# ActiveVisionLab/NeFeS

Measured on AMD Instinct MI355X. Metric: rays/s (fwd+bwd) at 640x480x(64+128) samples, 8x256 MLP, higher is better.
Workload: dtype f32; 1 GPU; BASELINE configs[1]: 7-Scenes-stairs geometry, 64+128 samples, 8x256 MLP + 16-ch feature head; 640x480, random seed-0 weights, fwd + bwd to the 3x4 pose; parallelism=rows/1

## Files before the change

include/nefes_hip.h:

```cpp
#ifndef NEFES_HIP_H
#define NEFES_HIP_H
#include <stddef.h>
#include <stdint.h>

#ifdef __cplusplus
extern "C" {
#endif

#define NEFES_ABI_VERSION 20
#define NEFES_BLOB_FORMAT 17

#define NEFES_E_BADARG (-1)
#define NEFES_E_UNSUPPORTED (-2)
#define NEFES_E_BADBLOB (-3)

typedef struct NefesNetDesc {
    int32_t width;
    int32_t feat_dim;
    int32_t has_transient;
    int32_t xyz_encoding;
    int32_t fold_final;
} NefesNetDesc;
#define NEFES_XYZ_FREQ10 0
#define NEFES_XYZ_EXTERNAL32 1
// ... 13 lines not shown
} NefesBlobInfo;

#define NEFES_COMP_TRANSIENT 1u
#define NEFES_COMP_STATIC_ONLY 2u
#define NEFES_COMP_SIGMA_ONLY 4u
#define NEFES_COMP_WHITE_BKGD 8u
#define NEFES_COMP_FEAT_WEIGHTS_ONLY 16u

#define NEFES_FIELD_SIGMA 0
#define NEFES_FIELD_STATIC 1
#define NEFES_FIELD_FULL 2

int nefes_version(void);

int nefes_blob_info(const NefesNetDesc* desc, NefesBlobInfo* info);
size_t nefes_stream_slab_bytes(const NefesNetDesc* desc, int stream);
int nefes_pack_weights(const NefesNetDesc* desc, const float* const* tensors, int n_tensors, void* blob,
                       size_t blob_bytes);
int nefes_pack_map(const NefesNetDesc* desc, uint32_t* map, size_t n_entries, int64_t* tensor_elems_out);
int nefes_pack_h3_plan(const NefesNetDesc* desc, int32_t* plan, size_t n_ints, size_t* needed);
int nefes_pack_device(const float* flat, int64_t n_params, const uint32_t* map, int64_t n_entries, const int32_t* plan,
                      int n_jobs, int32_t* scratch, void* blob, void* stream);

int nefes_raygen_fwd(int H, int W, float focal, const float* c2w, int row0, int nrows, float* rays_o, float* rays_d,
                     float* viewdirs, void* stream);
size_t nefes_raygen_bwd_workspace(int n_rays);
int nefes_raygen_bwd(int H, int W, float focal, const float* c2w, int row0, int nrows, const float* g_rays_o,
                     const float* g_rays_d, const float* g_viewdirs, void* workspace, float* g_c2w, void* stream);
int nefes_raygen_k_fwd(int H, int W, const float* intr, const float* c2w, int row0, int nrows, float* rays_o, float* rays_d,
                       float* viewdirs, void* stream);
// ... 280 lines not shown
```

nefes_amd/csrc/field_fwd_h3.hip:

```cpp
#include "field_h3_instances.h"
#ifdef NEFES_TU_W128
#define NEFES_SLAB_KIB 16
#else
#define NEFES_SLAB_KIB 32
#endif
#include <stdio.h>
#include <stdlib.h>
#if defined(NEFES_TU_W128) || !defined(H3_NO_ACC_READ_ASM)
#define NEFES_ASM_READS_ACC
#define NEFES_FENCE_TILES
#endif
#if defined(NEFES_TU_W128)
#define NEFES_ACC_VGPR_FORM
#endif

#ifndef NEFES_FWD_CONSUMER_BIAS
#define NEFES_FWD_CONSUMER_BIAS 1
#endif
#include "field_common.h"
#include "../../include/nefes_hip.h"

#include "field_x6.h"
#include "hashgrid.h"
#if !defined(NEFES_TU_W128) && !defined(H3_NO_ACC_READ_ASM)
#define H3_ACC_READ_ASM
#endif
#include "field_h3.h"
#define NEFES_H3_SLOTS 2

struct FieldFwdH3Args {
    const char* stream;
    const float* bias;
// ... 4 lines not shown
    const float* pts;
    const float* xyz_enc;
    const float* viewdirs;
    float* raw_t;
    uint32_t* masks;
    int N, S, R, C;
    long long M;
    int n_tiles;
    uint32_t s_magic, s_shift;
    float* acts;
    int rows;
    int z_row;
    const float2* hg_table;
    HgGeom hg;
    int gout;
};

template <int NT, int T0, int NX>
__device__ __forceinline__ void train_save_h3(float* tile_base, uint32_t voff, int row0, const f32x16 (&X)[NX], float inv) {
    float* p = tile_base + (size_t)(row0 >> 5) * 4096 + voff;
#pragma unroll
    for (int t = 0; t < NT; ++t)
#pragma unroll
        for (int r = 0; r < 16; ++r) {
#ifndef NEFES_TRAIN_NO_STORES
            __builtin_nontemporal_store(X[T0 + t][r] * inv, &p[t * 4096 + nefes_rho(0, r) * 16]);
#endif
        }
}

template <int MODEF, int ENC, int W = 256, int NTR = 1, bool TRAIN = false, bool FH = false>
__global__ __launch_bounds__(256, W == 128 ? 2 : 1) void field_fwd_h3_kernel(FieldFwdH3Args a) {
    constexpr bool FOLD = MODEF == NEFES_FIELD_FULL_FOLD;
    constexpr int MODE = FOLD ? NEFES_FIELD_FULL : MODEF;
    static_assert(NEFES_SLAB_KIB == (W == 128 ? NEFES_H3_FWD_SLAB_KIB_128 : NEFES_H3_FWD_SLAB_KIB), "ring slab size != the packer's for this width");
    static_assert(!FOLD || (MODE != NEFES_FIELD_SIGMA && !TRAIN), "the fold serves the head products of frozen networks");
    constexpr int NTW = W / 32, NTH = W / 64;
    constexpr int ES = ENC != NEFES_XYZ_FREQ10 ? NEFES_X_STEPS : NEFES_E_STEPS;
    constexpr int MW = 8 * (W / 64) + 4 * (W / 128), WT = (NTW + 1) / 2, WH = (NTH + 1) / 2;
    constexpr int NSEG = MODE == NEFES_FIELD_SIGMA ? NEFES_H3F_SIG + 1
                         : (MODE == NEFES_FIELD_STATIC ? NEFES_H3F_N_STATIC : (FOLD ? NEFES_H3FF_N : NEFES_H3F_N));
    extern __shared__ __attribute__((aligned(16))) char smem[];
    char* ring_base = smem;
    float* bias_lds = (float*)(smem + NEFES_H3_SLOTS * NEFES_SLAB_BYTES);
    float* e_lds = bias_lds + ((a.bias_floats + 63) / 64) * 64 + (threadIdx.x >> 6) * (ES * 64) + (threadIdx.x & 63);
    const int lane = threadIdx.x & 63;
    const int wave = __builtin_amdgcn_readfirstlane(threadIdx.x >> 6);
    const int j = lane & 31, h = lane >> 5;
    for (uint32_t i = threadIdx.x; i < a.bias_floats; i += 256) bias_lds[i] = a.bias[i];
    HgGeom* hg_lds = (HgGeom*)(bias_lds + ((a.bias_floats + 63) / 64) * 64 + 4 * ES * 64);
    if constexpr (ENC == NEFES_XYZ_HASHGRID_FUSED) {
        if (threadIdx.x == 0) *hg_lds = a.hg;
    }
    StagedRing ring;
    ring.init(a.stream, a.n_slabs, ring_base, wave, lane);
    const char* ring_lane = ring_base + lane * 16;
    const char* bias_half = (const char*)bias_lds + 16 * h;
    const int* tab_i = (const int*)(bias_lds + a.scale_off);
    const float* tab_f = bias_lds + a.scale_off;
    auto wexp = [&](int seg) { return tab_i[nefes_h3_tab_exp(nefes_h3f_seg(FOLD, seg))]; };
    auto rowb = [&](int seg) { return tab_f[nefes_h3_tab_bound(nefes_h3f_seg(FOLD, seg))]; };
    auto bmax = [&](int blk) { return tab_f[nefes_h3_tab_bias(NSEG, nefes_h3f_bias(FOLD, blk))]; };
    ring.prime(ring_lane);
    constexpr int B_SIG = 8 * W, B_FINAL = B_SIG + 32, B_DIR = B_FINAL + (FOLD ? 0 : W), B_RGB = B_DIR + W / 2,
                  B_T0 = B_RGB + 32 * NTR, B_T1 = B_T0 + W / 2, B_T2 = B_T1 + W / 2, B_TH = B_T2 + W / 2;
#pragma unroll 1
    for (int tile = blockIdx.x; tile < a.n_tiles; tile += gridDim.x) {
        auto locate = [&](uint32_t& m, uint32_t& ray, uint32_t& smp) {
            const uint32_t m_raw = (uint32_t)tile * 128u + (uint32_t)(wave * 32 + j);
            const bool ok = m_raw < (uint32_t)a.M;
            m = ok ? m_raw : (uint32_t)a.M - 1u;
            ray = a.s_magic ? __umulhi(m, a.s_magic) >> a.s_shift : m;
// ... 59 lines not shown
        };
        auto bias_at = [&](int off_floats, int es) { return BiasInitScaled{bias_half + off_floats * 4, pow2i(es)}; };
        constexpr bool CB = !TRAIN && W == 256 && NEFES_FWD_CONSUMER_BIAS;
        float2 nbias;
        f32x16 A[NTW], B[NTW];
        uint32_t bits[WT];
        auto clear_bits = [&]() {
#pragma unroll
            for (int w = 0; w < WT; ++w) bits[w] = 0u;
        };
        constexpr bool CAP = MODE != NEFES_FIELD_SIGMA;
        auto tau_of = [&](float M, int ew) {
            const int t = pick_exp(M);
            return t < 100 - ew ? t : 100 - ew;
        };
        auto sigma_head = [&](const f32x16 (&X)[NTW], int es_x, int tau_x) {
            f32x16 sg[1];
            float mdummy = 0.f;
            const int es = tau_x + wexp(NEFES_H3F_SIG);
            if constexpr (CB) {
                const char* bp8 = bias_half + 7 * W * 4;
                nbias = ReluBiasSplitH<false, NTW, WT>::prime(bp8);
                mma_run_h3<1, W / 16, 0, true>(ring, ring_lane, ReluBiasSplitH<false, NTW, WT>{X, bits, pow2i(tau_x - es_x), mdummy, bp8, pow2i(es_x), nbias},
                                               bias_at(B_SIG, es), sg);
            } else
            mma_run_h3<1, W / 16, 0, true>(ring, ring_lane, ReluSplitH<false, NTW, WT>{X, bits, pow2i(tau_x - es_x), mdummy},
                                           bias_at(B_SIG, es), sg);
            float* col = raw_col();
            if (col && h == 0) {
                const int ch = (MODE == NEFES_FIELD_SIGMA) ? 0 : 3 + a.C;
                __builtin_nontemporal_store(softplus_ref(sg[0][0] * pow2i(-es)), &col[(size_t)ch * a.S]);
            }
        };
        int es_a, es_b = 0;
        float M;
        {
            const int tau = tau_of(mE, wexp(NEFES_H3F_L1));
            es_a = tau + wexp(NEFES_H3F_L1);
            if constexpr (CB) mma_run_h3<NTW, ES / 8, 0, true>(ring, ring_lane, LdsSplitH{e_lds, pow2i(tau)}, ZeroInit{}, A);
            else mma_run_h3<NTW, ES / 8, 0, true>(ring, ring_lane, LdsSplitH{e_lds, pow2i(tau)}, bias_at(0, es_a), A);
            M = rowb(NEFES_H3F_L1) * mE + bmax(NEFES_H3BB_L1);
            save_trunk(1, A, es_a);
        }
#define NEFES_FWD_EVEN_LAYER(L1_, SEG1_)                                                                                       \
        clear_bits();                                                                                                          \
        {                                                                                                                      \
            const int ew = wexp(SEG1_), tau = tau_of(M, ew);                                                                   \
// ... 68 lines not shown
#pragma unroll
                for (int s = 0; s < NEFES_D_STEPS; ++s) __builtin_nontemporal_store(Dv[s], &pd[2 * s * 16]);
            }
            f32x16 dt[NDT];
            uint32_t bits2[WH];
            auto clear2 = [&]() {
#pragma unroll
                for (int w = 0; w < WH; ++w) bits2[w] = 0u;
            };
            struct Bias2 {
                BiasInitScaled a, b;
                __device__ __forceinline__ f32x16 operator()(int t) const { return t < NTH ? a(t) : b(t - NTH); }
            };
            int es_dt;
            if constexpr (FOLD) {
                sigma_head(B, es_b, tau_of(M, wexp(NEFES_H3F_SIG)));
                const int ew = wexp(NEFES_H3F_DT_H);
                const float mD = pair_max(array_max(Dv));
                const int tau = tau_of(fmaxf(M, mD), ew);
                const float rbh_ = rowb(NEFES_H3F_DT_H), rbd_ = rowb(NEFES_H3F_DT_D);
                const float bm_ = fmaxf(bmax(NEFES_H3BB_DIR), bmax(NEFES_H3BB_T0));
                float mx = 0.f;
                es_dt = tau + ew;
                clear_bits();
                if constexpr (CB) {
                    const char* bp8 = bias_half + 7 * W * 4;
                    nbias = ReluBiasSplitH<CAP, NTW, WT>::prime(bp8);
                    const ReluBiasSplitH<CAP, NTW, WT> src8{B, bits, pow2i(tau - es_b), mx, bp8, pow2i(es_b), nbias};
                    mma_run_h3<NDT, W / 16, 0, true>(ring, ring_lane, src8, Bias2{bias_at(B_DIR, es_dt), bias_at(B_T0, es_dt)}, dt);
                } else {
                    const ReluSplitH<CAP, NTW, WT> src8{B, bits, pow2i(tau - es_b), mx};
                    mma_run_h3<NDT, W / 16, 0, true>(ring, ring_lane, src8, Bias2{bias_at(B_DIR, es_dt), bias_at(B_T0, es_dt)}, dt);
                }
                mma_run_h3<NDT, 2, 0, false>(ring, ring_lane, ArraySplitH<16>{Dv, pow2i(tau)}, ZeroInit{}, dt);
                M = rbh_ * (pair_max(mx) * pow2i(-es_b)) + rbd_ * mD + bm_;
                put_masks(bits, WT);
            } else {
                const int ew = wexp(NEFES_H3F_DT_H);
                const float mD = pair_max(array_max(Dv));
                const int tau = tau_of(fmaxf(M, mD), ew);
                float mx = 0.f;
                es_dt = tau + ew;
                if constexpr (CB) {
                    const char* bpf = bias_half + B_FINAL * 4;
                    nbias = ReluBiasSplitH<false, 1, 1>::prime(bpf);
                    const IdentBiasSplitH<NTW> srcf{A, pow2i(tau - es_a), mx, bpf, pow2i(es_a), nbias};
                    if constexpr (FULL) mma_run_h3<NDT, W / 16, 0, true>(ring, ring_lane, srcf, Bias2{bias_at(B_DIR, es_dt), bias_at(B_T0, es_dt)}, dt);
                    else mma_run_h3<NDT, W / 16, 0, true>(ring, ring_lane, srcf, bias_at(B_DIR, es_dt), dt);
// ... 110 lines not shown
}

static void magic_div(uint32_t d, uint32_t& magic, uint32_t& shift) {
    if (d == 1) { magic = 0; shift = 0; return; }
    uint32_t l = 0;
    while ((1ull << l) < d) ++l;
    const uint64_t p = 31 + l;
    magic = (uint32_t)(((1ull << p) + d - 1) / d);
    shift = (uint32_t)(p - 32);
}

template <int MODE, int ENC, int W = 256, int NTR = 1, bool TRAIN = false, bool FH = false>
static int launch_h3(const FieldFwdH3Args& a, hipStream_t st) {
    constexpr int ES_ = ENC != NEFES_XYZ_FREQ10 ? NEFES_X_STEPS : NEFES_E_STEPS;
    const size_t lds = (size_t)NEFES_H3_SLOTS * NEFES_SLAB_BYTES + ((a.bias_floats + 63) / 64) * 256 + (size_t)4 * ES_ * 64 * 4
                       + (ENC == NEFES_XYZ_HASHGRID_FUSED ? 512 : 0);
    static_assert(sizeof(HgGeom) <= 512, "the level geometry's LDS slot");
    auto k = field_fwd_h3_kernel<MODE, ENC, W, NTR, TRAIN, FH>;
    hipError_t e = hipFuncSetAttribute((const void*)k, hipFuncAttributeMaxDynamicSharedMemorySize, (int)lds);
    if (e != hipSuccess) return (int)e;
    int dev = 0, cus = 256;
    (void)hipGetDevice(&dev);
    (void)hipDeviceGetAttribute(&cus, hipDeviceAttributeMultiprocessorCount, dev);
    const int per_cu = W == 128 ? 2 : 1;
    int grid = a.n_tiles < cus * per_cu ? a.n_tiles : cus * per_cu;
    if (const char* cap = getenv("NEFES_DEBUG_MAX_GRID")) {
        const int c = atoi(cap);
        if (c > 0 && c < grid) grid = c;
    }
    hipLaunchKernelGGL(k, dim3(grid), dim3(256), lds, st, a);
    return (int)hipGetLastError();
// ... 59 lines not shown
    } else {
        ok = (w == 256 || (w == 128 && !ext)) && cls >= 0 && (ext || desc->xyz_encoding == NEFES_XYZ_FREQ10);
        ok = ok && !(mode == NEFES_FIELD_STATIC && ext);
        ok = ok && !(fold && mode != NEFES_FIELD_SIGMA && !(mode == NEFES_FIELD_FULL && w == 256 && !ext && !fh));
        ok = ok && !(fh && (desc->feat_dim != 0 || w != 128 || ext || mode != NEFES_FIELD_FULL));
    }
    if (!ok) return {NEFES_E_UNSUPPORTED, nullptr};
    const NefesH3FwdKey key = {fold && mode == NEFES_FIELD_FULL ? NEFES_FIELD_FULL_FOLD : mode,
                               fused_grid ? NEFES_XYZ_HASHGRID_FUSED : desc->xyz_encoding, w,
                               mode == NEFES_FIELD_SIGMA ? (w == 128 ? 5 : 1) : (cls == 0 ? 1 : 5), train, fh};
    for (const H3FwdRow& r : h3_fwd_rows)
        if (r.key == key) return {0, &r};
    return {NEFES_E_UNSUPPORTED, nullptr};
}

static int h3_fwd_stream(const NefesNetDesc* desc, const NefesH3FwdKey& k, NefesStreamInfo* si) {
    NefesBlobInfo info;
    int rc = nefes_blob_info(desc, &info);
    if (rc) return rc;
    *si = info.stream[k.mode == NEFES_FIELD_SIGMA ? NEFES_STREAM_FWD_SIGMA_H3
                      : (k.mode == NEFES_FIELD_STATIC ? NEFES_STREAM_FWD_STATIC_H3 : NEFES_STREAM_FWD_FULL_H3)];
    return si->n_slabs == 0 ? NEFES_E_UNSUPPORTED : 0;
}

static int h3_fwd_args(const NefesNetDesc* desc, const void* packed, const NefesH3FwdKey& k, int N, int S,
                       const NefesHashGridDesc* grid, FieldFwdH3Args& a) {
    NefesStreamInfo si;
    int rc = h3_fwd_stream(desc, k, &si);
    if (rc) return rc;
    a.stream = (const char*)packed + si.slab_off;
    a.bias = (const float*)((const char*)packed + si.bias_off);
    a.n_slabs = si.n_slabs; a.bias_floats = si.bias_floats; a.scale_off = si.scale_off;
    if (k.enc == NEFES_XYZ_HASHGRID_FUSED) {
        rc = hg_geometry(grid, &a.hg, nullptr);
        if (rc) return rc;
        if (a.hg.n_levels != 16) return NEFES_E_UNSUPPORTED;
    }
    a.gout = k.fh ? k.w / 2 : 0;
    a.N = N; a.S = S; a.C = k.fh ? a.gout + 1 : desc->feat_dim;
    a.R = k.mode == NEFES_FIELD_SIGMA ? 1 : 3 + a.C + (k.mode == NEFES_FIELD_STATIC ? 1 : 6);
    a.M = (long long)N * S;
    if (a.M >= (1ll << 31) - 256) return NEFES_E_UNSUPPORTED;
    a.n_tiles = (int)((a.M + 127) / 128);
    a.rows = k.train ? nefes_train_row(desc->width, desc->feat_dim, NEFES_TB_END) : 0;
// ... 13 lines not shown

extern "C" int nefes_field_h3_instance(const NefesNetDesc* desc, int backward, int mode, unsigned request_flags, char* name, size_t cap) {
    if (!desc || !name || cap == 0) return NEFES_E_BADARG;
    name[0] = 0;
    const unsigned kind = request_flags & ~(unsigned)NEFES_H3_REQ_EXT;
    if ((kind & (kind - 1)) || (request_flags >> 6) || ((request_flags & NEFES_H3_REQ_EXT) && kind != NEFES_H3_REQ_TRAIN) ||
        (request_flags & (backward ? NEFES_H3_REQ_ZROW : NEFES_H3_REQ_STATIC_BWD)))
        return NEFES_E_BADARG;
    const char* text = nullptr;
    int rc;
    if (backward) {
        rc = nefes_h3_bwd_instance(desc, mode, request_flags, &text);
    } else {
        const H3FwdSel s = h3_fwd_select(desc, mode, request_flags);
        NefesStreamInfo si;
        rc = s.rc ? s.rc : h3_fwd_stream(desc, s.row->key, &si);
        if (!rc) text = s.row->name;
    }
    if (text) snprintf(name, cap, "%s", text);
    return rc;
}

extern "C" int nefes_field_fwd_train_h3(const NefesNetDesc* desc, const void* packed, int mode, int N, int S, const float* rays_o,
                                        const float* rays_d, const float* z, const float* pts, const float* viewdirs,
                                        float* raw_t, float* acts, uint32_t* masks, void* stream) {
    if (!desc || !packed || !raw_t || !acts || !viewdirs || N <= 0 || S <= 0) return NEFES_E_BADARG;
    if (!pts && !(rays_o && rays_d && z)) return NEFES_E_BADARG;
    FieldFwdH3Args a = {};
    a.rays_o = rays_o; a.rays_d = rays_d; a.z = z; a.pts = pts; a.viewdirs = viewdirs; a.raw_t = raw_t; a.masks = masks; a.acts = acts;
    return h3_fwd_run(desc, packed, mode, NEFES_H3_REQ_TRAIN, N, S, nullptr, a, stream);
}
// ... 58 lines not shown
```

nefes_amd/csrc/field_h3.h:

```cpp
#pragma once
#ifndef NEFES_H3_WIDE_MIN
#define NEFES_H3_WIDE_MIN 8
#endif
#ifndef NEFES_H3_WIDE_MAX
#define NEFES_H3_WIDE_MAX 64
#endif

typedef _Float16 f16x8 __attribute__((ext_vector_type(8)));

struct Split2 {
    u32x4 h, l;
};
__device__ __forceinline__ f16x8 as_f16x8(u32x4 v) {
    f16x8 r;
    __builtin_memcpy(&r, &v, 16);
    return r;
}
__device__ __forceinline__ f16x8 as_f16x8(f32x4 v) {
    f16x8 r;
    __builtin_memcpy(&r, &v, 16);
    return r;
}

__device__ __forceinline__ float pow2i(int e) {
// ... 313 lines not shown
        load_piece(q);
        if (q == NEFES_SLAB_PIECES - 1) g_next = (g_next + 1 == n_slabs) ? 0 : g_next + 1;
    }
    __device__ __forceinline__ uint32_t acquire() {
        asm volatile("s_waitcnt lgkmcnt(0)" ::: "memory");
        __builtin_amdgcn_s_barrier();
        c_slot ^= 1u;
        return c_slot * NEFES_SLAB_BYTES;
    }
    __device__ __forceinline__ void prime(const char* ring_lane) {
        asm volatile("s_waitcnt lgkmcnt(0)" ::: "memory");
        __builtin_amdgcn_s_barrier();
        cur_off = 0;
        pf = *(const f32x4*)(ring_lane);
    }
    __device__ __forceinline__ void drain() {}
};

__device__ __forceinline__ void mfma_h3_asm(f32x16& c, const f32x4& a, const u32x4& b) {
    asm volatile("v_mfma_f32_32x32x16_f16 %0, %1, %2, %0" : "+a"(c) : "v"(a), "v"(b));
}
__device__ __forceinline__ void mfma_h3_asm_v(f32x16& c, const f32x4& a, const u32x4& b) {
    asm volatile("v_mfma_f32_32x32x16_f16 %0, %1, %2, %0" : "+v"(c) : "v"(a), "v"(b));
}
__device__ __forceinline__ void mfma_h3_asm_c0(f32x16& c, const f32x4& a, const u32x4& b) {
    asm volatile("v_mfma_f32_32x32x16_f16 %0, %1, %2, 0" : "=a"(c) : "v"(a), "v"(b));
}
__device__ __forceinline__ void mfma_h3_asm_v_c0(f32x16& c, const f32x4& a, const u32x4& b) {
    asm volatile("v_mfma_f32_32x32x16_f16 %0, %1, %2, 0" : "=v"(c) : "v"(a), "v"(b));
}
template <class T> struct h3_is_zero_init { static constexpr bool value = false; };
template <> struct h3_is_zero_init<ZeroInit> { static constexpr bool value = true; };
// ... 10 lines not shown
    auto BQ = [&](int k) -> Split2& { return (k & 1) ? B1 : B0; };
    asm volatile("s_nop 13" ::: "memory");
#ifdef H3_WIDE_ENTRY_FENCE
    __builtin_amdgcn_sched_barrier(0);
    asm volatile("s_nop 7\n\ts_nop 7\n\ts_nop 1" ::: "memory");
    __builtin_amdgcn_sched_barrier(0);
#endif
    {
        PairRegs s0;
#pragma unroll
        for (int pp = 0; pp < 4; ++pp) {
            src.stage_a(s0, 0, pp);
            src.stage_b(s0);
            if (pp == 3) src.template stage_c<true>(B0, pp, s0);
            else src.template stage_c<false>(B0, pp, s0);
        }
    }
    constexpr bool C0 = FIRST && h3_is_zero_init<InitFn>::value
        ;
    if (FIRST && !C0) acc[T0] = init(0);
    const char* p = ring_lane + ring.cur_off;
    f32x4 ha0 = ring.pf, la0 = *(const f32x4*)(p + 1024);
    f32x4 ha1 = *(const f32x4*)(p + 2048), la1 = *(const f32x4*)(p + 3072);
    f32x4 ha2, la2;
    auto HA = [&](int k) -> f32x4& { return k % 3 == 0 ? ha0 : (k % 3 == 1 ? ha1 : ha2); };
    auto LA = [&](int k) -> f32x4& { return k % 3 == 0 ? la0 : (k % 3 == 1 ? la1 : la2); };
    PairRegs ps[4];
#pragma unroll
    for (int sl = 0; sl < NSLAB; ++sl) {
        const int nu = (NU - sl * UPS) < UPS ? (NU - sl * UPS) : UPS;
// ... 22 lines not shown
                        else asm volatile("s_nop 1" : "+a"(acc[T0 + t]));
                    }
                    if (vt) mfma_h3_asm_v(acc[T0 + t], l0, B.h);
                    else mfma_h3_asm(acc[T0 + t], l0, B.h);
                }
                __builtin_amdgcn_sched_barrier(0);
                if (host) src.stage_a(ps[pp], q + 1, pp);
                if (tail) src.template stage_c2<false>(Bn, pp, ps[pp]);
                if (!host && uu != acq_u) h2 = *(const f32x4*)(pn);
                __builtin_amdgcn_sched_barrier(0);
                asm volatile("" ::"v"(l0), "v"(B.h));
                if (vt) mfma_h3_asm_v(acc[T0 + t], h0, B.l);
                else mfma_h3_asm(acc[T0 + t], h0, B.l);
                __builtin_amdgcn_sched_barrier(0);
                if (host) src.stage_b(ps[pp]);
                if (host && uu != acq_u) h2 = *(const f32x4*)(pn);
                if (!host) {
#pragma unroll
                    for (int qq = 0; qq < NEFES_SLAB_PIECES; ++qq)
                        if (piece_unit(qq) == uu) ring.store_piece(qq);
                }
                if (FIRST && !C0 && q == 0 && t + 1 < NT) {
                    acc[T0 + t + 1] = init(t + 1);
                }
                __builtin_amdgcn_sched_barrier(0);
                asm volatile("" ::"v"(B.l));
                if (vt) mfma_h3_asm_v(acc[T0 + t], h0, B.h);
                else mfma_h3_asm(acc[T0 + t], h0, B.h);
                __builtin_amdgcn_sched_barrier(0);
                if (host) src.stage_c1(Bn, pp, ps[pp]);
// ... 31 lines not shown
__device__ __forceinline__ void mma_run_h3_small(Ring& ring, const char* ring_lane, const SrcFn& src, const InitFn& init,
                                           f32x16 (&acc)[NACC]) {
    static_assert(T0 + NT <= NACC, "accumulator array too small");
    constexpr int UPS = (NEFES_SLAB_FRAGS / 4) / 2;
    constexpr int NU = KS16 * NT;
    constexpr int NSLAB = (NU + UPS - 1) / UPS;
    Split2 B, Bn;
    {
        PairRegs s0;
#pragma unroll
        for (int pp = 0; pp < 4; ++pp) {
            src.stage_a(s0, 0, pp);
            src.stage_b(s0);
            if (pp == 3) src.template stage_c<true>(B, pp, s0);
            else src.template stage_c<false>(B, pp, s0);
        }
    }
    Bn = B;
    if (FIRST) acc[T0] = init(0);
    const char* p = ring_lane + ring.cur_off;
    f32x4 ah = ring.pf, al = *(const f32x4*)(p + 1024);
#pragma unroll
    for (int sl = 0; sl < NSLAB; ++sl) {
        const int nu = (NU - sl * UPS) < UPS ? (NU - sl * UPS) : UPS;
#pragma unroll
        for (int uu = 0; uu < UPS; ++uu) {
            if (uu < nu) {
                const int u = sl * UPS + uu, q = u / NT, t = u % NT;
                f32x4 nh;
                const bool last = !(uu + 1 < nu);
// ... 25 lines not shown
                        }
                }
                c = __builtin_amdgcn_mfma_f32_32x32x16_f16(Ah, Bl, c, 0, 0, 0);
                c = __builtin_amdgcn_mfma_f32_32x32x16_f16(Ah, Bh, c, 0, 0, 0);
                acc[T0 + t] = c;
                if (q + 1 < KS16) {
                    constexpr int STRIDE = NT >= 8 ? 2 : 1;
#pragma unroll
                    for (int pp = 0; pp < 4; ++pp)
                        if (NT >= 4 ? (t == pp * STRIDE + STRIDE - 1) : (t == (pp * NT) / 4)) {
                            PairRegs s1;
                            src.stage_a(s1, q + 1, pp);
                            src.stage_b(s1);
                            if (pp == 3) src.template stage_c<true>(Bn, pp, s1);
                            else src.template stage_c<false>(Bn, pp, s1);
#pragma unroll
                            for (int i = 0; i < 2; ++i) {
                                __builtin_amdgcn_sched_group_barrier(0x008, 1, 0);
                                __builtin_amdgcn_sched_group_barrier(0x002, 4, 0);
                            }
                        }
                }
                ah = nh;
            }
        }
    }
    ring.pf = ah;
    mfma_results_fence_tiles<12, NT, T0>(acc);
}

// ... 7 lines not shown
```

nefes_amd/csrc/layout.h:

```cpp
#pragma once
#include <stdint.h>

#if defined(__HIP__)
#define NEFES_HD __host__ __device__ inline __attribute__((always_inline))
#else
#define NEFES_HD inline
#endif

#ifndef NEFES_FWD_SLAB_KIB
#define NEFES_FWD_SLAB_KIB 32
#endif
#ifndef NEFES_BWD_SLAB_KIB
#define NEFES_BWD_SLAB_KIB 32
#endif
#define NEFES_FRAGS_OF_KIB(kib) ((kib) * 4)
#define NEFES_SLAB_BYTES (NEFES_SLAB_KIB * 1024)
#define NEFES_SLAB_FRAGS NEFES_FRAGS_OF_KIB(NEFES_SLAB_KIB)
#define NEFES_SLAB_PIECES (NEFES_SLAB_BYTES / 4096)
#define NEFES_RING_SLOTS (128 / NEFES_FWD_SLAB_KIB)
#define NEFES_BWD_SLOTS (96 / NEFES_BWD_SLAB_KIB)
#define NEFES_N_FREQ_XYZ 10
#define NEFES_N_FREQ_DIR 4
#define NEFES_E_STEPS 32
#define NEFES_D_STEPS 14
// ... 56 lines not shown
NEFES_HD int nefes_h3b_seg(int has_transient, int seg) { return (has_transient || seg == NEFES_H3B_RGB) ? seg : seg - 4; }
enum { NEFES_H3FF_SIG = NEFES_H3F_SIG, NEFES_H3FF_DT_H, NEFES_H3FF_DT_D, NEFES_H3FF_RGB, NEFES_H3FF_T1, NEFES_H3FF_T2, NEFES_H3FF_TH,
       NEFES_H3FF_N };
enum { NEFES_H3FBB_SIG = NEFES_H3BB_SIG, NEFES_H3FBB_DIR, NEFES_H3FBB_RGB, NEFES_H3FBB_T0, NEFES_H3FBB_T1, NEFES_H3FBB_T2, NEFES_H3FBB_TH };
enum { NEFES_H3BF_RGB = 0, NEFES_H3BF_TH, NEFES_H3BF_T2, NEFES_H3BF_T1, NEFES_H3BF_T0, NEFES_H3BF_DIR, NEFES_H3BF_SIG, NEFES_H3BF_L8,
       NEFES_H3BF_L7, NEFES_H3BF_L6, NEFES_H3BF_L5, NEFES_H3BF_L4, NEFES_H3BF_L3, NEFES_H3BF_L2, NEFES_H3BF_L1, NEFES_H3BF_N };
#define NEFES_H3FF_N_STATIC (NEFES_H3FF_RGB + 1)
#define NEFES_H3BF_N_STATIC (NEFES_H3BF_N - 4)
NEFES_HD int nefes_h3f_seg(int fold, int seg) { return (fold && seg > NEFES_H3F_FINAL) ? seg - 1 : seg; }
NEFES_HD int nefes_h3f_bias(int fold, int block) { return (fold && block > NEFES_H3BB_FINAL) ? block - 1 : block; }
NEFES_HD int nefes_h3b_fold_seg(int fold, int seg) { return (fold && seg > NEFES_H3B_FINAL) ? seg - 1 : seg; }
static_assert(NEFES_H3FF_DT_H == NEFES_H3F_DT_H - 1 && NEFES_H3FF_TH == NEFES_H3F_TH - 1 && NEFES_H3FBB_DIR == NEFES_H3BB_DIR - 1 &&
              NEFES_H3FBB_TH == NEFES_H3BB_TH - 1 && NEFES_H3BF_SIG == NEFES_H3B_SIG - 1 && NEFES_H3BF_L1 == NEFES_H3B_L1 - 1,
              "folded ordinals = the unfolded ones with FINAL taken out");

NEFES_HD int nefes_mask_words(int W) { return 8 * (W / 64) + 4 * (W / 128); }

enum { NEFES_TB_E = 0, NEFES_TB_DV = 1, NEFES_TB_L1 = 2 , NEFES_TB_FINAL = 10, NEFES_TB_DIR = 11,
       NEFES_TB_T0 = 12, NEFES_TB_T1 = 13, NEFES_TB_T2 = 14, NEFES_TB_RGB = 15, NEFES_TB_SIG = 16, NEFES_TB_TH = 17,
       NEFES_TB_END = 18 };
NEFES_HD size_t nefes_train_off(int row, int sample) {
    return ((size_t)(row >> 5) * 8 + (size_t)(sample >> 4)) * 512 + (size_t)(row & 31) * 16 + (size_t)(sample & 15);
}
NEFES_HD uint32_t nefes_train_lane_off(int wave, int j, int h) { return (uint32_t)(((wave * 32 + j) >> 4) * 512 + 4 * h * 16 + (j & 15)); }
NEFES_HD int nefes_train_row(int W, int C, int block) {
    const int ntr = nefes_head_ntr(C);
    int r = 0;
    if (block == NEFES_TB_E) return r;
    r += 2 * NEFES_E_STEPS;
    if (block == NEFES_TB_DV) return r;
// ... 13 lines not shown
```

nefes_amd/csrc/pack.cpp:

```cpp
#include <math.h>
#include <string.h>

#include <vector>

#include "../../include/nefes_hip.h"
#include "layout.h"

namespace {

enum { L_XYZ1 = 0, L_FINAL = 8, L_DIR = 9, L_SIGMA = 10, L_RGB = 11, L_T0 = 12, L_T1 = 13, L_T2 = 14, L_TSIGMA = 15,
       L_TRGB = 16, L_TBETA = 17 };

struct Seg {
    int nt = 0, ks = 0;
    std::vector<int> kidx;
    std::vector<int> ridx;
    const float* W = nullptr;
    int ld = 0;
    bool transposed = false;
    bool x6 = false;
    bool h3 = false;
    int wexp = 0;
    float at(int s, int t, int lane) const {
        const int i = lane & 31, h = lane >> 5;
// ... 506 lines not shown
}

extern "C" int nefes_version(void) { return NEFES_ABI_VERSION; }

extern "C" size_t nefes_stream_slab_bytes(const NefesNetDesc* desc, int stream) {
    if (!desc || stream < 0 || stream >= 13) return 0;
    return (size_t)nefes_stream_slab_kib(stream, desc->width) * 1024;
}

extern "C" int nefes_blob_info(const NefesNetDesc* desc, NefesBlobInfo* info) {
    if (!desc || !info) return NEFES_E_BADARG;
    Net n;
    Stream st[NEFES_N_STREAMS];
    if (!build(desc, nullptr, n, st)) return NEFES_E_UNSUPPORTED;
    fill_info(st, desc->width, info);
    return 0;
}

static int64_t tensor_elems(const Net& n, int i) {
    const int l = i / 2;
    const bool bias = i & 1;
    int out, in;
    if (l < 8) { out = n.W; in = l == 0 ? n.in_xyz : (l == 4 ? n.in_xyz + n.W : n.W); }
    else if (l == L_FINAL) { out = n.W; in = n.W; }
    else if (l == L_DIR || l == L_T0) { out = n.W2; in = n.W + 27; }
    else if (l == L_SIGMA) { out = 1; in = n.W; }
    else if (l == L_RGB) { out = 3 + n.C; in = n.W2; }
    else if (l == L_T1 || l == L_T2) { out = n.W2; in = n.W2; }
    else if (l == L_TRGB) { out = 3; in = n.W2; }
    else { out = 1; in = n.W2; }
// ... 249 lines not shown
```

nefes_amd/lib.py:

```python
import ctypes as C
import os

import torch

_HERE = os.path.dirname(os.path.abspath(__file__))
LIB_PATH = os.environ.get("NEFES_HIP_LIB") or os.path.join(_HERE, "libnefes_hip.so")


class NefesNetDesc(C.Structure):
    _fields_ = [("width", C.c_int32), ("feat_dim", C.c_int32), ("has_transient", C.c_int32), ("xyz_encoding", C.c_int32),
                ("fold_final", C.c_int32)]


class NefesGenericNetDesc(C.Structure):
    _fields_ = [("width", C.c_int32), ("depth", C.c_int32), ("skip", C.c_int32), ("feat_dim", C.c_int32), ("has_transient", C.c_int32),
                ("xyz_encoding", C.c_int32)]


class NefesStreamInfo(C.Structure):
    _fields_ = [("slab_off", C.c_uint64), ("n_slabs", C.c_uint32), ("bias_floats", C.c_uint32), ("bias_off", C.c_uint64),
                ("scale_off", C.c_uint32), ("scale_count", C.c_uint32)]


class NefesBlobInfo(C.Structure):
# ... 20 lines not shown
                                                                                              17, 18)
COMP_TRANSIENT, COMP_STATIC_ONLY, COMP_SIGMA_ONLY, COMP_WHITE_BKGD, COMP_FEAT_WEIGHTS_ONLY = 1, 2, 4, 8, 16

TRAIN_LOSS_ROWS = 16
LOSS_FEAT_MSE, LOSS_FEAT_L1, LOSS_FEAT_COS = 0, 1, 2
(LOSS_HAS_RGB_FINE, LOSS_HAS_RGB_COARSE, LOSS_HAS_BETA, LOSS_HAS_FEAT_FINE, LOSS_HAS_FEAT_COARSE, LOSS_HAS_FEAT_FUSION,
 LOSS_NERFW) = 1, 2, 4, 8, 16, 32, 64

_p, _i, _f, _u32, _sz = C.c_void_p, C.c_int, C.c_float, C.c_uint32, C.c_size_t
_desc = C.POINTER(NefesNetDesc)
_gdesc = C.POINTER(NefesGenericNetDesc)

SIGNATURES = {
    "nefes_version": (_i, []),
    "nefes_blob_info": (_i, [_desc, C.POINTER(NefesBlobInfo)]),
    "nefes_stream_slab_bytes": (_sz, [_desc, _i]),
    "nefes_fusion_input_fwd": (_i, [_i, _i, _i, _p, _p, _p, C.POINTER(_f), C.POINTER(_f), _p, _p, _p]),
    "nefes_fusion_input_bwd": (_i, [_i, _i, _i, _p, _p, _p, C.POINTER(_f), _p, _p, _p]),
    "nefes_upcos_loss_fwd": (_i, [_i, _i, _i, _i, _i, _i, _p, _p, _p, _p, _p]),
    "nefes_upcos_loss_bwd": (_i, [_i, _i, _i, _i, _i, _i, _p, _p, _p, _p, _p, _p, _p, _p, _p, _p, _i, _p, _p, _p]),
    "nefes_bicubic_gather_table": (_i, [_i, _i, _i, _i, _i, _p, _p, _p, _p]),
    "nefes_bicubic_gram": (_i, [_i, _i, _i, _i, _p, _p]),
    "nefes_bn_train_fwd": (_i, [_i, _i, C.c_int64, _i, _p, _p, _p, C.c_double, C.c_double, _p, _p, _p, _p, _p, _p]),
    "nefes_bn_train_bwd": (_i, [_i, _i, C.c_int64, _i, _p, _p, _p, _p, _p, _p]),
    "nefes_bn_train_bwd_affine": (_i, [_i, _i, C.c_int64, _p, _p, _p, _p, _p, _p, _p, _p]),
    "nefes_svd_reg_fwd": (_i, [_i, _p, _p, _p, _p]),
    "nefes_svd_reg_bwd": (_i, [_i, _p, _p, _p, _p]),
    "nefes_regressed_pose_fwd": (_i, [_i, _p, _i, _f, _f, _f, _f, _p, _p, _p]),
    "nefes_regressed_pose_bwd": (_i, [_i, _p, _i, _f, _p, _p, _p]),
    "nefes_upcos_prepare": (_i, [_i, _i, _i, _i, _i, _i, _p, _p, _p, _p, _p, _p, _p, _i, _p, _p, _p, _p]),
# ... 138 lines not shown
```

Measured before the change: 766,200 rays/s.

## Compute sigma head as FP32 dot product riding the fused MMA pass

Replaces the sigma head's single-output MFMA tile (a 32-wide matmul used for a 1-wide output) with a per-lane FP32 dot product against a sigma weight row staged in LDS. The row comes from the backward-static stream. In the folded full-field path the dot is accumulated inside the next MMA run's staging loop through a DotRide wrapper, so the activations are read only once. The ring skips the now-unused sigma slab with step_over. This costs extra LDS, a permlane swap reduction and extra VALU FMAs inside the MFMA loop, and it changes numerics slightly because the sigma product is now FP32 rather than FP16 MFMA.

```diff
diff --git a/include/nefes_hip.h b/include/nefes_hip.h
--- a/include/nefes_hip.h
+++ b/include/nefes_hip.h
@@ -51,6 +51,7 @@
 int nefes_version(void);
 
 int nefes_blob_info(const NefesNetDesc* desc, NefesBlobInfo* info);
+int nefes_h3_sigma_row(const NefesNetDesc* desc, NefesBlobInfo* info, uint64_t* byte_off);
 size_t nefes_stream_slab_bytes(const NefesNetDesc* desc, int stream);
 int nefes_pack_weights(const NefesNetDesc* desc, const float* const* tensors, int n_tensors, void* blob,
                        size_t blob_bytes);
diff --git a/nefes_amd/csrc/field_fwd_h3.hip b/nefes_amd/csrc/field_fwd_h3.hip
--- a/nefes_amd/csrc/field_fwd_h3.hip
+++ b/nefes_amd/csrc/field_fwd_h3.hip
@@ -16,6 +16,12 @@
 
 #ifndef NEFES_FWD_CONSUMER_BIAS
 #define NEFES_FWD_CONSUMER_BIAS 1
+#endif
+#ifndef NEFES_SIGMA_DOT
+#define NEFES_SIGMA_DOT 1
+#endif
+#ifndef NEFES_SIGMA_RIDE
+#define NEFES_SIGMA_RIDE 1
 #endif
 #include "field_common.h"
 #include "../../include/nefes_hip.h"
@@ -50,6 +56,7 @@
     const float2* hg_table;
     HgGeom hg;
     int gout;
+    const float* sig_row;
 };
 
 template <int NT, int T0, int NX>
@@ -79,12 +86,15 @@
     extern __shared__ __attribute__((aligned(16))) char smem[];
     char* ring_base = smem;
     float* bias_lds = (float*)(smem + NEFES_H3_SLOTS * NEFES_SLAB_BYTES);
-    float* e_lds = bias_lds + ((a.bias_floats + 63) / 64) * 64 + (threadIdx.x >> 6) * (ES * 64) + (threadIdx.x & 63);
+    constexpr int ROWF = NEFES_SIGMA_DOT ? W : 0;
+    float* row_lds = bias_lds + ((a.bias_floats + 63) / 64) * 64;
+    float* e_lds = row_lds + ROWF + (threadIdx.x >> 6) * (ES * 64) + (threadIdx.x & 63);
     const int lane = threadIdx.x & 63;
     const int wave = __builtin_amdgcn_readfirstlane(threadIdx.x >> 6);
     const int j = lane & 31, h = lane >> 5;
     for (uint32_t i = threadIdx.x; i < a.bias_floats; i += 256) bias_lds[i] = a.bias[i];
-    HgGeom* hg_lds = (HgGeom*)(bias_lds + ((a.bias_floats + 63) / 64) * 64 + 4 * ES * 64);
+    for (int i = threadIdx.x; i < ROWF; i += 256) row_lds[i] = a.sig_row[nefes_sigma_row_word(i)];
+    HgGeom* hg_lds = (HgGeom*)(row_lds + ROWF + 4 * ES * 64);
     if constexpr (ENC == NEFES_XYZ_HASHGRID_FUSED) {
         if (threadIdx.x == 0) *hg_lds = a.hg;
     }
@@ -92,6 +102,7 @@
     ring.init(a.stream, a.n_slabs, ring_base, wave, lane);
     const char* ring_lane = ring_base + lane * 16;
     const char* bias_half = (const char*)bias_lds + 16 * h;
+    const char* row_half = (const char*)row_lds + 16 * h;
     const int* tab_i = (const int*)(bias_lds + a.scale_off);
     const float* tab_f = bias_lds + a.scale_off;
     auto wexp = [&](int seg) { return tab_i[nefes_h3_tab_exp(nefes_h3f_seg(FOLD, seg))]; };
@@ -181,9 +192,28 @@
             const int t = pick_exp(M);
             return t < 100 - ew ? t : 100 - ew;
         };
+        auto sigma_store = [&](float dot, int es_x) {
+            const float pre = add_rn(bias_lds[B_SIG], mul_rn(dot, pow2i(-es_x)));
+            float* col = raw_col();
+            if (col && h == 0) {
+                const int ch = (MODE == NEFES_FIELD_SIGMA) ? 0 : 3 + a.C;
+                __builtin_nontemporal_store(softplus_ref(pre), &col[(size_t)ch * a.S]);
+            }
+        };
         auto sigma_head = [&](const f32x16 (&X)[NTW], int es_x, int tau_x) {
+            float mdummy = 0.f;
+#if NEFES_SIGMA_DOT
+            ring.step_over(ring_lane);
+            float dot;
+            if constexpr (CB) {
+                const char* bp8 = bias_half + 7 * W * 4;
+                nbias = ReluBiasSplitH<false, NTW, WT>::prime(bp8);
+                dot = dot_row_h3<W / 16>(ReluBiasSplitH<false, NTW, WT>{X, bits, 1.f, mdummy, bp8, pow2i(es_x), nbias}, row_half);
+            } else
+                dot = dot_row_h3<W / 16>(ReluSplitH<false, NTW, WT>{X, bits, 1.f, mdummy}, row_half);
+            sigma_store(dot, es_x);
+#else
             f32x16 sg[1];
-            float mdummy = 0.f;
             const int es = tau_x + wexp(NEFES_H3F_SIG);
             if constexpr (CB) {
                 const char* bp8 = bias_half + 7 * W * 4;
@@ -198,6 +228,7 @@
                 const int ch = (MODE == NEFES_FIELD_SIGMA) ? 0 : 3 + a.C;
                 __builtin_nontemporal_store(softplus_ref(sg[0][0] * pow2i(-es)), &col[(size_t)ch * a.S]);
             }
+#endif
         };
         int es_a, es_b = 0;
         float M;
@@ -296,6 +327,12 @@
             };
             int es_dt;
             if constexpr (FOLD) {
+                constexpr bool RIDE = NEFES_SIGMA_DOT && NEFES_SIGMA_RIDE;
+                DotRowH3 sdot;
+                if constexpr (RIDE) {
+                    ring.step_over(ring_lane);
+                    sdot.begin(row_half);
+                } else
                 sigma_head(B, es_b, tau_of(M, wexp(NEFES_H3F_SIG)));
                 const int ew = wexp(NEFES_H3F_DT_H);
                 const float mD = pair_max(array_max(Dv));
@@ -309,11 +346,20 @@
                     const char* bp8 = bias_half + 7 * W * 4;
                     nbias = ReluBiasSplitH<CAP, NTW, WT>::prime(bp8);
                     const ReluBiasSplitH<CAP, NTW, WT> src8{B, bits, pow2i(tau - es_b), mx, bp8, pow2i(es_b), nbias};
+                    if constexpr (RIDE)
+                        mma_run_h3<NDT, W / 16, 0, true>(ring, ring_lane, DotRideH<ReluBiasSplitH<CAP, NTW, WT>>{src8, sdot},
+                                                         Bias2{bias_at(B_DIR, es_dt), bias_at(B_T0, es_dt)}, dt);
+                    else
                     mma_run_h3<NDT, W / 16, 0, true>(ring, ring_lane, src8, Bias2{bias_at(B_DIR, es_dt), bias_at(B_T0, es_dt)}, dt);
                 } else {
                     const ReluSplitH<CAP, NTW, WT> src8{B, bits, pow2i(tau - es_b), mx};
+                    if constexpr (RIDE)
+                        mma_run_h3<NDT, W / 16, 0, true>(ring, ring_lane, DotRideH<ReluSplitH<CAP, NTW, WT>>{src8, sdot},
+                                                         Bias2{bias_at(B_DIR, es_dt), bias_at(B_T0, es_dt)}, dt);
+                    else
                     mma_run_h3<NDT, W / 16, 0, true>(ring, ring_lane, src8, Bias2{bias_at(B_DIR, es_dt), bias_at(B_T0, es_dt)}, dt);
                 }
+                if constexpr (RIDE) sigma_store(sdot.end(), es_b);
                 mma_run_h3<NDT, 2, 0, false>(ring, ring_lane, ArraySplitH<16>{Dv, pow2i(tau)}, ZeroInit{}, dt);
                 M = rbh_ * (pair_max(mx) * pow2i(-es_b)) + rbd_ * mD + bm_;
                 put_masks(bits, WT);
@@ -454,7 +500,7 @@
 static int launch_h3(const FieldFwdH3Args& a, hipStream_t st) {
     constexpr int ES_ = ENC != NEFES_XYZ_FREQ10 ? NEFES_X_STEPS : NEFES_E_STEPS;
     const size_t lds = (size_t)NEFES_H3_SLOTS * NEFES_SLAB_BYTES + ((a.bias_floats + 63) / 64) * 256 + (size_t)4 * ES_ * 64 * 4
-                       + (ENC == NEFES_XYZ_HASHGRID_FUSED ? 512 : 0);
+                       + (ENC == NEFES_XYZ_HASHGRID_FUSED ? 512 : 0) + (NEFES_SIGMA_DOT ? (size_t)W * 4 : 0);
     static_assert(sizeof(HgGeom) <= 512, "the level geometry's LDS slot");
     auto k = field_fwd_h3_kernel<MODE, ENC, W, NTR, TRAIN, FH>;
     hipError_t e = hipFuncSetAttribute((const void*)k, hipFuncAttributeMaxDynamicSharedMemorySize, (int)lds);
@@ -544,9 +590,9 @@
     return {NEFES_E_UNSUPPORTED, nullptr};
 }
 
-static int h3_fwd_stream(const NefesNetDesc* desc, const NefesH3FwdKey& k, NefesStreamInfo* si) {
+static int h3_fwd_stream(const NefesNetDesc* desc, const NefesH3FwdKey& k, NefesStreamInfo* si, uint64_t* sig_row_off) {
     NefesBlobInfo info;
-    int rc = nefes_blob_info(desc, &info);
+    int rc = nefes_h3_sigma_row(desc, &info, sig_row_off);
     if (rc) return rc;
     *si = info.stream[k.mode == NEFES_FIELD_SIGMA ? NEFES_STREAM_FWD_SIGMA_H3
                       : (k.mode == NEFES_FIELD_STATIC ? NEFES_STREAM_FWD_STATIC_H3 : NEFES_STREAM_FWD_FULL_H3)];
@@ -556,8 +602,10 @@
 static int h3_fwd_args(const NefesNetDesc* desc, const void* packed, const NefesH3FwdKey& k, int N, int S,
                        const NefesHashGridDesc* grid, FieldFwdH3Args& a) {
     NefesStreamInfo si;
-    int rc = h3_fwd_stream(desc, k, &si);
+    uint64_t sig_row_off = 0;
+    int rc = h3_fwd_stream(desc, k, &si, &sig_row_off);
     if (rc) return rc;
+    a.sig_row = (const float*)((const char*)packed + sig_row_off);
     a.stream = (const char*)packed + si.slab_off;
     a.bias = (const float*)((const char*)packed + si.bias_off);
     a.n_slabs = si.n_slabs; a.bias_floats = si.bias_floats; a.scale_off = si.scale_off;
@@ -601,7 +649,8 @@
     } else {
         const H3FwdSel s = h3_fwd_select(desc, mode, request_flags);
         NefesStreamInfo si;
-        rc = s.rc ? s.rc : h3_fwd_stream(desc, s.row->key, &si);
+        uint64_t sig_row_off;
+        rc = s.rc ? s.rc : h3_fwd_stream(desc, s.row->key, &si, &sig_row_off);
         if (!rc) text = s.row->name;
     }
     if (text) snprintf(name, cap, "%s", text);
diff --git a/nefes_amd/csrc/field_h3.h b/nefes_amd/csrc/field_h3.h
--- a/nefes_amd/csrc/field_h3.h
+++ b/nefes_amd/csrc/field_h3.h
@@ -351,8 +351,72 @@
         cur_off = 0;
         pf = *(const f32x4*)(ring_lane);
     }
+    __device__ __forceinline__ void step_over(const char* ring_lane) {
+#pragma unroll
+        for (int q = 0; q < NEFES_SLAB_PIECES; ++q) issue_piece(q);
+        cur_off = acquire();
+        pf = *(const f32x4*)(ring_lane + cur_off);
+    }
     __device__ __forceinline__ void drain() {}
 };
+
+__device__ __forceinline__ float pair_sum(float v) {
+    const uint32_t u = __float_as_uint(v);
+    const auto r = __builtin_amdgcn_permlane32_swap(u, u, false, false);
+    return __uint_as_float(r[0]) + __uint_as_float(r[1]);
+}
+
+struct DotRowH3 {
+    const char* wp;
+    float s[8];
+    float2 nw;
+    __device__ __forceinline__ void begin(const char* wp_) {
+        wp = wp_;
+#pragma unroll
+        for (int i = 0; i < 8; ++i) s[i] = 0.f;
+        nw = *(const float2*)(wp + ReluBiasSplitH<false, 1, 1>::pair_off(0, 0));
+    }
+    __device__ __forceinline__ void pair(const PairRegs& x, int q, int p) {
+        const float2 w = nw;
+        const int qn = p == 3 ? q + 1 : q, pn = p == 3 ? 0 : p + 1;
+        nw = *(const float2*)(wp + ReluBiasSplitH<false, 1, 1>::pair_off(qn, pn));
+        s[2 * p] = __builtin_fmaf(w.x, x.x0, s[2 * p]);
+        s[2 * p + 1] = __builtin_fmaf(w.y, x.x1, s[2 * p + 1]);
+    }
+    __device__ __forceinline__ float end() const {
+        return pair_sum(((s[0] + s[1]) + (s[2] + s[3])) + ((s[4] + s[5]) + (s[6] + s[7])));
+    }
+};
+template <int KS16, class SrcFn>
+__device__ __forceinline__ float dot_row_h3(const SrcFn& src, const char* wp) {
+    DotRowH3 dot;
+    dot.begin(wp);
+#pragma unroll
+    for (int q = 0; q < KS16; ++q)
+#pragma unroll
+        for (int p = 0; p < 4; ++p) {
+            PairRegs x;
+            src.stage_a(x, q, p);
+            src.stage_b(x);
+            dot.pair(x, q, p);
+        }
+    return dot.end();
+}
+template <class Base>
+struct DotRideH {
+    Base b;
+    DotRowH3& dot;
+    __device__ __forceinline__ void stage_a(PairRegs& s, int q, int p) const { b.stage_a(s, q, p); }
+    __device__ __forceinline__ void stage_b(PairRegs& s) const { b.stage_b(s); }
+    template <bool NOP>
+    __device__ __forceinline__ void stage_c(Split2& o, int p, const PairRegs& s) const { b.template stage_c<NOP>(o, p, s); }
+    __device__ __forceinline__ void stage_c1(Split2& o, int p, const PairRegs& s) const { b.stage_c1(o, p, s); }
+    template <bool NOP>
+    __device__ __forceinline__ void stage_c2(Split2& o, int p, const PairRegs& s) const { b.template stage_c2<NOP>(o, p, s); }
+    __device__ __forceinline__ void stage_d(const PairRegs& s, int q, int p) const { dot.pair(s, q, p); }
+};
+template <class T> struct h3_rides_dot { static constexpr bool value = false; };
+template <class B> struct h3_rides_dot<DotRideH<B>> { static constexpr bool value = true; };
 
 __device__ __forceinline__ void mfma_h3_asm(f32x16& c, const f32x4& a, const u32x4& b) {
     asm volatile("v_mfma_f32_32x32x16_f16 %0, %1, %2, %0" : "+a"(c) : "v"(a), "v"(b));
@@ -393,6 +457,7 @@
             src.stage_b(s0);
             if (pp == 3) src.template stage_c<true>(B0, pp, s0);
             else src.template stage_c<false>(B0, pp, s0);
+            if constexpr (h3_rides_dot<SrcFn>::value) src.stage_d(s0, 0, pp);
         }
     }
     constexpr bool C0 = FIRST && h3_is_zero_init<InitFn>::value
@@ -445,6 +510,9 @@
                 else mfma_h3_asm(acc[T0 + t], h0, B.l);
                 __builtin_amdgcn_sched_barrier(0);
                 if (host) src.stage_b(ps[pp]);
+                if constexpr (h3_rides_dot<SrcFn>::value) {
+                    if (tail) src.stage_d(ps[pp], q + 1, pp);
+                }
                 if (host && uu != acq_u) h2 = *(const f32x4*)(pn);
                 if (!host) {
 #pragma unroll
@@ -506,6 +574,7 @@
             src.stage_b(s0);
             if (pp == 3) src.template stage_c<true>(B, pp, s0);
             else src.template stage_c<false>(B, pp, s0);
+            if constexpr (h3_rides_dot<SrcFn>::value) src.stage_d(s0, 0, pp);
         }
     }
     Bn = B;
@@ -561,6 +630,7 @@
                             src.stage_b(s1);
                             if (pp == 3) src.template stage_c<true>(Bn, pp, s1);
                             else src.template stage_c<false>(Bn, pp, s1);
+                            if constexpr (h3_rides_dot<SrcFn>::value) src.stage_d(s1, q + 1, pp);
 #pragma unroll
                             for (int i = 0; i < 2; ++i) {
                                 __builtin_amdgcn_sched_group_barrier(0x008, 1, 0);
diff --git a/nefes_amd/csrc/layout.h b/nefes_amd/csrc/layout.h
--- a/nefes_amd/csrc/layout.h
+++ b/nefes_amd/csrc/layout.h
@@ -94,6 +94,8 @@
               NEFES_H3FBB_TH == NEFES_H3BB_TH - 1 && NEFES_H3BF_SIG == NEFES_H3B_SIG - 1 && NEFES_H3BF_L1 == NEFES_H3B_L1 - 1,
               "folded ordinals = the unfolded ones with FINAL taken out");
 
+NEFES_HD int nefes_sigma_row_word(int k) { return ((k >> 5) >> 2) * 256 + ((k >> 5) & 3) + 4 * (k & 31); }
+
 NEFES_HD int nefes_mask_words(int W) { return 8 * (W / 64) + 4 * (W / 128); }
 
 enum { NEFES_TB_E = 0, NEFES_TB_DV = 1, NEFES_TB_L1 = 2 , NEFES_TB_FINAL = 10, NEFES_TB_DIR = 11,
diff --git a/nefes_amd/csrc/pack.cpp b/nefes_amd/csrc/pack.cpp
--- a/nefes_amd/csrc/pack.cpp
+++ b/nefes_amd/csrc/pack.cpp
@@ -544,6 +544,27 @@
     Stream st[NEFES_N_STREAMS];
     if (!build(desc, nullptr, n, st)) return NEFES_E_UNSUPPORTED;
     fill_info(st, desc->width, info);
+    return 0;
+}
+
+extern "C" int nefes_h3_sigma_row(const NefesNetDesc* desc, NefesBlobInfo* info_out, uint64_t* byte_off) {
+    if (!desc || !byte_off) return NEFES_E_BADARG;
+    Net n;
+    Stream st[NEFES_N_STREAMS];
+    if (!build(desc, nullptr, n, st)) return NEFES_E_UNSUPPORTED;
+    NefesBlobInfo info;
+    fill_info(st, desc->width, &info);
+    if (info_out) *info_out = info;
+    const int k = NEFES_STREAM_BWD_STATIC_H3;
+    const Stream& s = st[k];
+    const int ord = nefes_h3b_seg(0, nefes_h3b_fold_seg(n.fold, NEFES_H3B_SIG));
+    if (info.stream[k].n_slabs == 0 || ord >= (int)s.segs.size()) return NEFES_E_UNSUPPORTED;
+    const Seg& sg = s.segs[ord];
+    if (sg.x6 || !sg.transposed || sg.ks != 1 || sg.nt != n.NTW || sg.ld != n.W) return NEFES_E_UNSUPPORTED;
+    const int frags = NEFES_FRAGS_OF_KIB(nefes_stream_slab_kib(k, desc->width));
+    uint64_t slab = 0;
+    for (int i = 0; i < ord; ++i) slab += (uint64_t)s.segs[i].slabs(frags);
+    *byte_off = info.stream[k].slab_off + slab * (uint64_t)frags * 256;
     return 0;
 }
 
diff --git a/nefes_amd/lib.py b/nefes_amd/lib.py
--- a/nefes_amd/lib.py
+++ b/nefes_amd/lib.py
@@ -58,6 +58,7 @@
 SIGNATURES = {
     "nefes_version": (_i, []),
     "nefes_blob_info": (_i, [_desc, C.POINTER(NefesBlobInfo)]),
+    "nefes_h3_sigma_row": (_i, [_desc, C.POINTER(NefesBlobInfo), C.POINTER(C.c_uint64)]),
     "nefes_stream_slab_bytes": (_sz, [_desc, _i]),
     "nefes_fusion_input_fwd": (_i, [_i, _i, _i, _p, _p, _p, C.POINTER(_f), C.POINTER(_f), _p, _p, _p]),
     "nefes_fusion_input_bwd": (_i, [_i, _i, _i, _p, _p, _p, C.POINTER(_f), _p, _p, _p]),
```

New measurement: 773,700 rays/s, median of 6. No clear change (+1.0%).
